# iden3/rapidsnark-old

Measured on AMD Instinct MI355X. Metric: Groth16 proofs/sec, higher is better.
Workload: dtype i64 (v_mad_i64_i32 column sums over 9x29-bit signed limbs, BN254 Fr/Fq)

## Files before the change

### include/zkhip.h

```cpp
#ifndef ZKHIP_H
#define ZKHIP_H

#include <stdint.h>
#include <stddef.h>

#ifdef __cplusplus
extern "C" {
#endif

typedef struct zk_prover zk_prover;

typedef struct zk_zkey_view {
    uint32_t nVars;
    uint32_t nPublic;
    uint32_t domainSize;
    uint64_t nCoefs;
    const void *vk_alpha1;
    const void *vk_beta1;
    const void *vk_beta2;
    const void *vk_delta1;
    const void *vk_delta2;
    const void *coefs;
    const void *pointsA;
    const void *pointsB1;
// ... 56 lines not shown
    uint32_t window_bits_w, windows_w;
    uint32_t precomputed_tables;
    uint32_t msm_a_b1_c_one_launch;
    uint32_t lanes;
    uint32_t follow_up_streams;
    uint32_t max_in_flight;
    uint32_t depth_host_witness;
    uint32_t depth_resident_witness;
    uint32_t batch;
    uint32_t shard_index, shard_count, chain_partitioned;
    uint64_t device_bytes_in_use;
    uint64_t device_bytes_total;
    uint64_t kernel_launches_last_proof;
    uint32_t table_rows_h, table_rows_w;
    uint32_t bucket_sets_h, bucket_sets_w;
} zk_prover_plan;
int zk_prover_info(zk_prover *p, zk_prover_plan *plan);
int zk_prove_msm_collect(zk_prover *p, zk_msm_sums *partial);
int zk_prove_batch_submit(zk_prover *p, const uint8_t *const *wtns, uint32_t count, const uint8_t *r32s, const uint8_t *s32s);
int zk_prove_batch_collect(zk_prover *p, zk_proof *out, uint32_t count);

int zk_prove_msm_dev(zk_prover *p, const void *d_wtns, zk_msm_sums *partial);
int zk_prove_msm(zk_prover *p, const uint8_t *wtns, zk_msm_sums *partial);
int zk_prove_finish(zk_prover *p, const zk_msm_sums *partials, uint32_t n_partials,
                    const uint8_t *r32, const uint8_t *s32, zk_proof *out);

typedef struct zk_multi_prover zk_multi_prover;
int zk_multi_prover_create(zk_multi_prover **out, const zk_zkey_view *zkey, const int32_t *devices, uint32_t n_devices,
                           const zk_opts *opts );
void zk_multi_prover_destroy(zk_multi_prover *mp);
// ... 103 lines not shown
```

### rapidsnark-old_amd/csrc/kernels.hpp

```cpp
#pragma once
#include <hip/hip_runtime.h>
#include <stdint.h>
#include "field.hpp"
#include "curve.hpp"

namespace zk {

void launch_fr_mul_vec(Fr *out, const Fr *a, const Fr *b, uint64_t n, hipStream_t s);
void launch_fq_mul_vec(Fq *out, const Fq *a, const Fq *b, uint64_t n, hipStream_t s);

struct CsrDev {
    const uint32_t *rowptr;
    const uint32_t *col;
    const Fr *val;
};
void launch_spmv_abc(Fr *a, Fr *b, Fr *c, CsrDev csr, const Fr *wtns, uint32_t n, hipStream_t s, uint32_t vectors = 1, uint64_t abc_stride = 0,
                     uint64_t wtns_stride = 0);
void launch_csr_build(uint32_t *rowptr, uint32_t *col, Fr *val, uint32_t *cursor, uint32_t *err, const uint8_t *records,
                      uint64_t nCoefs, uint32_t n, uint32_t nVars, uint32_t row_lo, uint32_t row_hi, hipStream_t s);
void launch_exclusive_scan_u32(uint32_t *out, const uint32_t *counts, uint32_t total, hipStream_t s);

struct TwEntry {
    uint32_t l[12];
};
// ... 2 lines not shown
    const TwEntry *fwd;
    const TwEntry *inv;
    const Fr *coset;
    const Fr *ninv;
};
struct NttPair {
    uint32_t L = 0, Lg = 0, m = 0;
    uint32_t ngroups = 0, g[2] = {0, 0};
    TwEntry *rfwd = nullptr, *rinv = nullptr;
    Fr *tinv = nullptr, *tfwd = nullptr, *dtab = nullptr, *t2inv = nullptr, *t2fwd = nullptr;
    NttPair() {}
    NttPair(const NttPair &) = delete;
    NttPair &operator=(const NttPair &) = delete;
    ~NttPair() { release(); }
    void build(uint32_t logn_global, uint32_t logn_local, uint32_t block_index, hipStream_t s, bool plain = false);
    void release();
};
bool ntt_pair_supported(uint32_t local_logn);
void launch_ntt_coset_pair(Fr *data, uint64_t stride_elems, uint32_t batch, const NttPair &t, hipStream_t s);
void launch_ntt_plain(Fr *out, Fr *data, uint64_t stride_elems, uint32_t batch, const NttPair &t, bool inverse, hipStream_t s);

void launch_ntt_build_tables(TwEntry *fwd, TwEntry *inv, Fr *coset, Fr *ninv, uint32_t logn, hipStream_t s);
#define NTT_FULL 0xffffffffu
void launch_ntt_dif_inverse(Fr *data, uint64_t stride_elems, uint32_t batch, const NttTables &t, hipStream_t s, uint32_t local_logn = NTT_FULL);
void launch_ntt_dit_forward(Fr *data, uint64_t stride_elems, uint32_t batch, const NttTables &t, hipStream_t s, const Fr *premul = nullptr,
                            uint32_t local_logn = NTT_FULL);
void launch_ntt_cross(bool inverse, const Fr *xb, uint64_t in_src_stride, uint64_t in_poly_stride, Fr *const out_base[8],
                      uint64_t out_poly_stride, uint64_t out_offset, uint32_t batch,
                      const NttTables &t, uint32_t log_shards, uint32_t rank, hipStream_t s);
void launch_chunk_scatter(Fr *const xb_of_gpu[8], const Fr *blockdata, uint32_t batch, uint32_t logn, uint32_t log_shards, uint32_t rank,
                          hipStream_t s);
void launch_chunk_pack(Fr *packed, const Fr *blockdata, uint32_t batch, uint32_t logn, uint32_t log_shards, hipStream_t s);
void launch_chunk_unpack(Fr *blockdata, const Fr *packed, uint32_t batch, uint32_t logn, uint32_t log_shards, hipStream_t s);
void launch_fr_to_internal(Fr *x, uint64_t n, int times, hipStream_t s);
// ... 81 lines not shown
```

### rapidsnark-old_amd/csrc/nttpair.hip

```cpp
#include <stdlib.h>
#include <string.h>
#include "kernels.hpp"
#include "hipcheck.hpp"
#include "common.hpp"
#include "field29.hpp"

namespace zk {

template <class F>
__device__ __forceinline__ F pload_el(const F *p) {
    const uint4 *q = reinterpret_cast<const uint4 *>(p);
    uint4 lo = q[0], hi = q[1];
    F r;
    r.v[0] = lo.x; r.v[1] = lo.y; r.v[2] = lo.z; r.v[3] = lo.w;
    r.v[4] = hi.x; r.v[5] = hi.y; r.v[6] = hi.z; r.v[7] = hi.w;
    return r;
}
template <class F>
__device__ __forceinline__ void pstore_el(F *p, const F &r) {
    uint4 *q = reinterpret_cast<uint4 *>(p);
    q[0] = make_uint4(r.v[0], r.v[1], r.v[2], r.v[3]);
    q[1] = make_uint4(r.v[4], r.v[5], r.v[6], r.v[7]);
}
__device__ __forceinline__ Fr29 pload_tw(const TwEntry *e) {
// ... 362 lines not shown
            const uint64_t i0 = i & (N1 - 1), k1 = pbrev((uint32_t)(i >> m), t);
            const uint64_t e = (i0 * k1) & (n - 1);
            pstore_el(tfwd + i, Fr29::store(Fr29::from_mont256(pfr_pow(s_wn, e))));
            pstore_el(tinv + i, Fr29::store(Fr29::from_mont256(Fr::mul(plain ? pfr_pow(s_wni, e) : Fr::mul(pfr_pow(s_wni, e), pfr_pow(s_w2n, k1)), s_kappa))));
        }
        if (t2fwd && i < (1ull << t)) {
            const uint32_t tb = t - ta;
            const uint64_t ja = i & ((1ull << ta) - 1), kb = pbrev((uint32_t)(i >> ta), tb);
            const uint64_t e = (ja * kb) & ((1ull << t) - 1);
            pstore_el(t2fwd + i, Fr29::store(Fr29::from_mont256(pfr_pow(s_wt, e))));
            pstore_el(t2inv + i, Fr29::store(Fr29::from_mont256(pfr_pow(s_wti, e))));
        }
    }
}

bool ntt_pair_supported(uint32_t local_logn) { return local_logn >= 3 && local_logn <= 27; }

void NttPair::build(uint32_t logn_global, uint32_t logn_local, uint32_t block_index, hipStream_t s, bool plain) {
    L = logn_local;
    Lg = logn_global;
    m = L < 11 ? L : 11;
    const uint32_t t = L - m;
    ngroups = t == 0 ? 0 : (t <= 11 ? 1 : 2);
    if (const char *e = probe_env("ZKHIP_NTT_SPLIT")) {
        if (atoi(e) == 2 && t >= 2) ngroups = 2;
    }
    g[0] = ngroups == 2 ? (t + 1) / 2 : t;
    g[1] = t - g[0];
    const uint64_t n = 1ull << L;
    auto dalloc = [&](void **p, size_t bytes) { ZK_HIP(hipMalloc(p, bytes ? bytes : 16)); };
// ... 5 lines not shown
        dalloc((void **)&tinv, n * sizeof(Fr));
        dalloc((void **)&tfwd, n * sizeof(Fr));
    }
    if (ngroups == 2) {
        dalloc((void **)&t2inv, ((size_t)1 << t) * sizeof(Fr));
        dalloc((void **)&t2fwd, ((size_t)1 << t) * sizeof(Fr));
    }
    const uint32_t lg = Lg - L;
    uint32_t rho = 0;
    for (uint32_t i = 0; i < lg; i++) rho |= ((block_index >> i) & 1u) << (lg - 1 - i);
    uint64_t grid = ((n > 2048 ? n : 2048) + 255) / 256;
    if (grid > 4096) grid = 4096;
    ZK_LAUNCH(k_pair_tables, dim3((uint32_t)grid), dim3(256), 0, s, rfwd, rinv, tinv, tfwd, dtab, t2inv, t2fwd, L, Lg, rho, m, g[0], plain ? 1u : 0u);
    ZK_LAUNCH_OK("ntt pair tables");
}
void NttPair::release() {
    for (void *p : {(void *)rfwd, (void *)rinv, (void *)tinv, (void *)tfwd, (void *)dtab, (void *)t2inv, (void *)t2fwd})
        if (p) (void)hipFree(p);
    rfwd = rinv = nullptr;
    tinv = tfwd = dtab = t2inv = t2fwd = nullptr;
}

static void lds_opt_in() {
    static PerDeviceOnce attr;
    if (!attr.need()) return;
    ZK_HIP(hipFuncSetAttribute((const void *)k_ntt_outer<true, 256>, hipFuncAttributeMaxDynamicSharedMemorySize, 160 * 1024));
    ZK_HIP(hipFuncSetAttribute((const void *)k_ntt_outer<false, 256>, hipFuncAttributeMaxDynamicSharedMemorySize, 160 * 1024));
    ZK_HIP(hipFuncSetAttribute((const void *)k_ntt_outer<true, 512>, hipFuncAttributeMaxDynamicSharedMemorySize, 160 * 1024));
    ZK_HIP(hipFuncSetAttribute((const void *)k_ntt_outer<false, 512>, hipFuncAttributeMaxDynamicSharedMemorySize, 160 * 1024));
    ZK_HIP(hipFuncSetAttribute((const void *)k_ntt_mid<0>, hipFuncAttributeMaxDynamicSharedMemorySize, 160 * 1024));
    ZK_HIP(hipFuncSetAttribute((const void *)k_ntt_mid<1>, hipFuncAttributeMaxDynamicSharedMemorySize, 160 * 1024));
// ... 57 lines not shown
            run_outer<true>(data, stride, batch, tb, tb.m + tb.g[0], tb.g[1], nullptr, 0, s);
            run_outer<true>(data, stride, batch, tb, tb.m, tb.g[0], tb.t2inv, t, s);
        } else if (tb.ngroups == 1) {
            run_outer<true>(data, stride, batch, tb, tb.m, t, nullptr, 0, s);
        }
    } else {
        if (tb.ngroups == 2) {
            run_outer<false>(data, stride, batch, tb, tb.m, tb.g[0], tb.t2fwd, t, s);
            run_outer<false>(data, stride, batch, tb, tb.m + tb.g[0], tb.g[1], nullptr, 0, s);
        } else if (tb.ngroups == 1) {
            run_outer<false>(data, stride, batch, tb, tb.m, t, nullptr, 0, s);
        }
    }
}

void launch_ntt_coset_pair(Fr *data, uint64_t stride, uint32_t batch, const NttPair &tb, hipStream_t s) {
    run_outer_passes<true>(data, stride, batch, tb, s);
    run_mid<0>(data, data, stride, batch, tb, s);
    run_outer_passes<false>(data, stride, batch, tb, s);
}

void launch_ntt_plain(Fr *out, Fr *data, uint64_t stride, uint32_t batch, const NttPair &tb, bool inverse, hipStream_t s) {
    if (inverse) {
        run_outer_passes<true>(data, stride, batch, tb, s);
        run_mid<1>(out, data, stride, batch, tb, s);
    } else {
        run_mid<2>(out, data, stride, batch, tb, s);
        run_outer_passes<false>(out, stride, batch, tb, s);
    }
}

}
```

### rapidsnark-old_amd/csrc/operators.hip

```cpp
#include "prover_internal.hpp"

static void need_device() { need_device_count(); }

template <class F>
static void mul_vec(uint8_t *out, const uint8_t *a, const uint8_t *b, uint64_t n, void (*launch)(F *, const F *, const F *, uint64_t, hipStream_t)) {
    need_device();
    if (!n) return;
    DevBuf<F> da, db;
    da.alloc(n);
    db.alloc(n);
    da.upload(a, n, 0);
    db.upload(b, n, 0);
    launch(da.p, da.p, db.p, n, 0);
    HIP_TRY(hipMemcpy(out, da.p, n * 32, hipMemcpyDeviceToHost));
}

struct Tables {
    DevBuf<TwEntry> fwd, inv;
    DevBuf<Fr> coset, ninv;
    NttTables t;
    void build(uint32_t logn) {
        uint64_t n = 1ull << logn;
        fwd.alloc(n > 1 ? n / 2 : 1);
        inv.alloc(n > 1 ? n / 2 : 1);
// ... 96 lines not shown
        need_device();
        uint32_t logn = ilog2_exact(n);
        if (logn > 27) throw std::invalid_argument("n exceeds 2^27");
        Tables tb;
        tb.build(logn);
        DevBuf<Fr> abc, hh;
        abc.alloc(3 * n);
        hh.alloc(n);
        HIP_TRY(hipMemcpy(abc.p, a, n * 32, hipMemcpyHostToDevice));
        HIP_TRY(hipMemcpy(abc.p + n, b, n * 32, hipMemcpyHostToDevice));
        launch_fr_mul_vec(abc.p + 2 * n, abc.p, abc.p + n, n, 0);
        launch_fr_to_internal(abc.p, 3 * n, 1, 0);
        if (ntt_pair_supported(logn) && !probe_env("ZKHIP_NTT_RADIX2")) {
            NttPair pr;
            pr.build(logn, logn, 0, 0);
            launch_ntt_coset_pair(abc.p, n, 3, pr, 0);
            HIP_TRY(hipStreamSynchronize(0));
        } else {
            launch_ntt_dif_inverse(abc.p, n, 3, tb.t, 0);
            launch_ntt_dit_forward(abc.p, n, 3, tb.t, 0, tb.coset.p);
        }
        launch_abc_to_h(hh.p, abc.p, abc.p + n, abc.p + 2 * n, n, 0);
        HIP_TRY(hipMemcpy(h, hh.p, n * 32, hipMemcpyDeviceToHost));
    });
}

}

template <class AffT, class XT, class AccT>
static void msm_generic(uint8_t *out, const uint8_t *bases, const uint8_t *scalars, uint64_t n, bool g2) {
    need_device();
// ... 103 lines not shown
```

### rapidsnark-old_amd/csrc/prover_create.hip

```cpp
#include "prover_internal.hpp"

__attribute__((constructor)) static void zk_default_hw_queues() { setenv("GPU_MAX_HW_QUEUES", "16", 0); }

namespace zkp {

void alloc_slot(zk_prover *p, int i) {
    zk_prover::ProofSlot &q = p->slot[i];
    if (q.allocated) return;
    const uint64_t nv = p->sv.size();
    q.sort_w.alloc(nv, p->wbits, p->table_mode, p->batch);
    const MsmPlan pw = q.sort_w.plan, ph = p->sort_h.plan;
    const uint64_t tbw = q.sort_w.total_buckets(), tbh = p->sort_h.total_buckets();
    q.buckets_g1.alloc(3 * tbw + tbh);
    q.buckets_g2.alloc(tbw);
    q.scratch_g1.alloc(msm_reduce_scratch_points(3, pw) + msm_reduce_scratch_points(1, ph));
    const uint64_t ew = (uint64_t)pw.sets * msm_wsum_rc(pw), eh = (uint64_t)ph.sets * msm_wsum_rc(ph);
    q.wsum_g1.alloc(3 * ew + eh);
    q.scratch_g2.alloc(msm_reduce_scratch_points(1, pw));
    q.wsum_g2.alloc(ew);
    const uint64_t slots = msm_accum_workspace_slots(q.sort_w.max_entries()), slots_h = msm_accum_workspace_slots(p->sort_h.max_entries());
    q.acc_stride = slots;
    q.acc_ws_g1_all.alloc(3 * slots + slots_h);
    q.acc_ws_g2.alloc(slots);
    q.acc_key_all.alloc(4 * slots + slots_h);
    q.acc_flag_all.alloc(4 * slots + slots_h);
    for (int m = 0; m < 5; m++) {
        const uint64_t at = m < 3 ? m * slots : (m == 3 ? 3 * slots : 3 * slots + slots_h);
        if (m < 4) q.acc_ws_g1[m] = q.acc_ws_g1_all.p + at;
        q.acc_key[m] = q.acc_key_all.p + at;
        q.acc_flag[m] = q.acc_flag_all.p + at;
    }
    q.w1_bytes = (size_t)(3 * ew + eh) * sizeof(G1XYZZ);
    q.w2_bytes = (size_t)ew * sizeof(G2XYZZ);
    if (!q.w1) HIP_TRY(hipHostMalloc((void **)&q.w1, q.w1_bytes, hipHostMallocDefault));
    if (!q.w2) HIP_TRY(hipHostMalloc((void **)&q.w2, q.w2_bytes, hipHostMallocDefault));
    for (auto &e : q.ev_l1)
        if (!e) HIP_TRY(hipEventCreateWithFlags(&e, hipEventDisableTiming));
    for (hipEvent_t *e : {&q.ev_fork, &q.ev_join, &q.ev_sortw, &q.ev_main, &q.ev_done, &q.ev_chain})
        if (!*e) HIP_TRY(hipEventCreateWithFlags(e, hipEventDisableTiming));
    for (auto &e : q.ev_tail)
        if (!e) HIP_TRY(hipEventCreateWithFlags(&e, hipEventDisableTiming));
    for (auto &e : q.ev)
        if (!e) HIP_TRY(hipEventCreate(&e));
    q.have_events = true;
    q.allocated = true;
}

void ensure_witness_buffer(zk_prover *p, zk_prover::ProofSlot &q) {
    if (!q.wtns_dev.p) q.wtns_dev.alloc((uint64_t)p->nVars * p->batch);
    if (!q.ev_h2d) HIP_TRY(hipEventCreateWithFlags(&q.ev_h2d, hipEventDisableTiming));
    if (!q.ev_h2d_start) HIP_TRY(hipEventCreate(&q.ev_h2d_start));
}

// ... 83 lines not shown
            {
                const char *e = getenv("ZKHIP_TAIL");
                int ntail = e ? atoi(e) : (p->shard_count > 1 ? 2 : 0);
                if (getenv("ZKHIP_SERIAL")) ntail = 0;
                if (ntail != 0 && ntail != 5) ntail = 2;
                p->tail_streams = ntail;
                if (ntail) {
                    int lo_pr = 0, hi_pr = 0;
                    HIP_TRY(hipDeviceGetStreamPriorityRange(&lo_pr, &hi_pr));
                    for (int i = 0; i < ntail; i++) HIP_TRY(hipStreamCreateWithPriority(&p->tail_pool[i], hipStreamNonBlocking, hi_pr));
                    for (int m = 0; m < 5; m++) p->tail[m] = ntail == 5 ? p->tail_pool[m] : p->tail_pool[(m == 2 || m == 3) ? 1 : 0];
                }
            }
            HIP_TRY(hipStreamCreateWithFlags(&p->stream_fin, hipStreamNonBlocking));
            HIP_TRY(hipStreamCreateWithFlags(&p->stream_h2d, hipStreamNonBlocking));
        } catch (...) {
            side.err = std::current_exception();
        }
    });
    p->wbits = (wbits == 0 && (p->flags & ZK_FLAG_SPARSE_WITNESS) && (p->flags & ZK_FLAG_PRECOMP) && p->logn > 18) ? 16u : wbits;
    hipStream_t s = p->stream;
    clk.lap("device + first stream", s);
    StreamUploader up(s);

    p->sv = shard_slice(nV, p->shard_index, p->shard_count);
    p->sh = shard_slice(n, p->shard_index, p->shard_count);
    p->part = (p->flags & ZK_FLAG_PARTITIONED_CHAIN) != 0 && p->shard_count > 1;
    if (p->part) {
        uint32_t lg = 0;
        while ((1u << lg) < p->shard_count) lg++;
// ... 25 lines not shown
        clk.lap("coefficient records upload", s);
        launch_csr_build(p->csr_rowptr.p, p->csr_col.p, p->csr_val.p, cursor.p, err.p, raw.p, nnz, z->domainSize, z->nVars,
                         p->part ? (uint32_t)p->sh.lo : 0u, p->part ? (uint32_t)p->sh.hi : z->domainSize, s);
        launch_fr_to_internal(p->csr_val.p, nnz, 2, s);
        uint32_t bad = 0;
        HIP_TRY(hipMemcpyAsync(&bad, err.p, 4, hipMemcpyDeviceToHost, s));
        HIP_TRY(hipStreamSynchronize(s));
        if (bad) throw std::invalid_argument("zkey coefficient record out of range");
        clk.lap("CSR build (device)", s);
    }

    {
        const uint32_t local_logn = p->logn - p->log_shards_chain();
        const bool pair = ntt_pair_supported(local_logn) && !probe_env("ZKHIP_NTT_RADIX2");
        if (pair) p->pair.build(p->logn, local_logn, p->part ? p->shard_index : 0u, s);
        if (!pair || p->part) {
            p->tw_fwd.alloc(n > 1 ? n / 2 : 1);
            p->tw_inv.alloc(n > 1 ? n / 2 : 1);
            if (!pair) p->tw_coset.alloc(n);
            p->tw_ninv.alloc(1);
            launch_ntt_build_tables(p->tw_fwd.p, p->tw_inv.p, p->tw_coset.p, p->tw_ninv.p, p->logn, s);
        }
    }
    clk.lap("twiddle tables", s);

    const uint64_t nv = p->sv.size(), nh = p->sh.size();
    p->precomp = (p->flags & ZK_FLAG_PRECOMP) != 0;
    p->table_mode = (p->flags & ZK_FLAG_PRECOMP_HALF) ? 2u : p->precomp ? 1u : 0u;
    p->sort_h.alloc(nh, wbits, p->table_mode, p->batch);
    alloc_slot(p.get(), 0);
// ... 179 lines not shown
        o.lanes = (uint32_t)p->lanes;
        o.follow_up_streams = (uint32_t)p->tail_streams;
        o.max_in_flight = ZK_MAX_IN_FLIGHT;
        const bool small = p->logn < 19, mid = p->logn <= 22 && p->shard_count == 1;
        o.depth_host_witness = small ? ZK_MAX_IN_FLIGHT : mid ? 6u : 3u;
        o.depth_resident_witness = small ? ZK_MAX_IN_FLIGHT : mid ? 6u : 2u;
        o.batch = p->batch;
        o.shard_index = p->shard_index; o.shard_count = p->shard_count; o.chain_partitioned = p->part ? 1u : 0u;
        {
            DeviceGuard g(p->device);
            size_t fr = 0, tot = 0;
            HIP_TRY(hipMemGetInfo(&fr, &tot));
            o.device_bytes_in_use = tot - fr; o.device_bytes_total = tot;
        }
        o.kernel_launches_last_proof = p->launches_last_proof;
        const uint32_t nb = plan->size < sizeof o ? plan->size : (uint32_t)sizeof o;
        o.size = nb;
        memcpy(plan, &o, nb);
    });
}

}
```

### rapidsnark-old_amd/csrc/prover_internal.hpp

```cpp
#pragma once
#include <hip/hip_runtime.h>
#include <string.h>
#include <stdio.h>
#include <stdlib.h>
#include <chrono>
#include <sys/random.h>
#include <string>
#include <vector>
#include <atomic>
#include <condition_variable>
#include <deque>
#include <map>
#include <mutex>
#include <thread>
#include <memory>
#include <stdexcept>
#include <exception>
#include <functional>

#include "../../include/zkhip.h"
#include "common.hpp"
#include "hipcheck.hpp"
#include "kernels.hpp"
#include "tail_pool.hpp"
// ... 144 lines not shown
struct zk_prover {
    int device = 0;
    uint32_t flags = 0;
    uint32_t nVars = 0, nPublic = 0, domainSize = 0, logn = 0;
    uint64_t nCoefs = 0;
    uint32_t shard_index = 0, shard_count = 1;
    uint8_t vk_alpha1[64], vk_beta1[64], vk_beta2[128], vk_delta1[64], vk_delta2[128];
    hipStream_t stream = nullptr, stream2 = nullptr;
    std::mutex mtx, cmtx, sync_mtx;

    DevBuf<uint32_t> csr_rowptr, csr_col;
    DevBuf<Fr> csr_val;
    DevBuf<TwEntry> tw_fwd, tw_inv;
    DevBuf<Fr> tw_coset, tw_ninv;
    NttPair pair;
    Slice sv, sh;
    uint32_t c_idx_min = 0;
    bool precomp = false;
    uint32_t table_mode = 0;
    DevBuf<G1Affine> ptsA, ptsB1, ptsC, ptsH;
    DevBuf<G2Affine> ptsB2;

    DevBuf<Fr> abc, h;
    SortBufs sort_h;
    struct ProofSlot {
        bool allocated = false, busy = false;
        bool use_tails = true;
        uint32_t l1_chunk_min = 0, l1_chunk_max = 0;
        SortBufs sort_w;
        DevBuf<G1Acc> buckets_g1;
        DevBuf<G2Acc> buckets_g2;
        DevBuf<G1Acc> scratch_g1, acc_ws_g1_all;
        G1Acc *acc_ws_g1[4] = {nullptr, nullptr, nullptr, nullptr};
        DevBuf<uint32_t> acc_key_all, acc_flag_all;
        uint32_t *acc_key[5] = {nullptr}, *acc_flag[5] = {nullptr};
        uint64_t acc_stride = 0;
        DevBuf<G2Acc> scratch_g2, acc_ws_g2;
        DevBuf<G1XYZZ> wsum_g1;
        DevBuf<G2XYZZ> wsum_g2;
        hipEvent_t ev_l1[5] = {nullptr, nullptr, nullptr, nullptr, nullptr};
        hipEvent_t ev_fork = nullptr, ev_join = nullptr, ev_sortw = nullptr, ev_main = nullptr, ev_done = nullptr, ev_chain = nullptr;
        bool zeroed = false;
        bool defer_w = false;
        hipEvent_t ev_tail[5] = {nullptr, nullptr, nullptr, nullptr, nullptr};
        hipEvent_t ev[20] = {};
        bool have_events = false;
        uint8_t *w1 = nullptr, *w2 = nullptr;
        size_t w1_bytes = 0, w2_bytes = 0;
        DevBuf<Fr> wtns_dev;
        uint8_t *wtns_pin = nullptr;
        uint8_t *pin_ring = nullptr;
        StageJob stage[ZK_MAX_BATCH];
        StageJob stage_chunk[16];
        hipEvent_t ev_h2d_b = nullptr;
        hipEvent_t ev_h2d = nullptr, ev_h2d_start = nullptr;
        uint8_t r32[ZK_MAX_BATCH][32], s32[ZK_MAX_BATCH][32];
        bool have_r = false, have_s = false;
// ... 15 lines not shown
            acc_key_all.release(); acc_flag_all.release(); scratch_g2.release(); acc_ws_g2.release();
            wsum_g1.release(); wsum_g2.release(); wtns_dev.release();
            if (w1) { (void)hipHostFree(w1); w1 = nullptr; }
            if (w2) { (void)hipHostFree(w2); w2 = nullptr; }
            if (wtns_pin) { (void)hipHostFree(wtns_pin); wtns_pin = nullptr; }
            if (pin_ring) { (void)hipHostFree(pin_ring); pin_ring = nullptr; }
            if (gexec) { (void)hipGraphExecDestroy(gexec); gexec = nullptr; }
            if (graph) { (void)hipGraphDestroy(graph); graph = nullptr; }
            graph_wtns = nullptr;
        }
        ~ProofSlot() {
            if (gexec) (void)hipGraphExecDestroy(gexec);
            if (graph) (void)hipGraphDestroy(graph);
            if (ev_gdone) (void)hipEventDestroy(ev_gdone);
            for (auto &e : ev_l1) if (e) (void)hipEventDestroy(e);
            for (hipEvent_t e : {ev_fork, ev_join, ev_sortw, ev_main, ev_done, ev_chain}) if (e) (void)hipEventDestroy(e);
            for (auto &e : ev_tail) if (e) (void)hipEventDestroy(e);
            for (auto &e : ev) if (e) (void)hipEventDestroy(e);
            if (w1) (void)hipHostFree(w1);
            if (w2) (void)hipHostFree(w2);
            if (wtns_pin) (void)hipHostFree(wtns_pin);
            if (pin_ring) (void)hipHostFree(pin_ring);
            if (ev_h2d) (void)hipEventDestroy(ev_h2d);
            if (ev_h2d_b) (void)hipEventDestroy(ev_h2d_b);
            if (ev_h2d_start) (void)hipEventDestroy(ev_h2d_start);
        }
    };
    ProofSlot slot[ZK_MAX_IN_FLIGHT];
    uint32_t next_submit = 0, next_collect = 0, in_flight = 0;
    uint32_t ring = ZK_MAX_IN_FLIGHT;
    uint32_t batch = 1;
// ... 38 lines not shown
    Fr *abc_use = nullptr, *xb_use = nullptr;
    Fr *pk_use = nullptr;
    Fr *peer_abc[8] = {nullptr}, *peer_xb[8] = {nullptr};
    bool have_peers = false;
    int phase_open = -1, phase_next = 0;
    hipEvent_t ev_ext_in = nullptr, ev_ext_out = nullptr;
    uint32_t log_shards_chain() const { return part ? log_shards : 0; }
    hipStream_t tail_pool[5] = {nullptr, nullptr, nullptr, nullptr, nullptr};
    hipStream_t tail[5] = {nullptr, nullptr, nullptr, nullptr, nullptr};
    int tail_streams = 0;
    bool use_graph = false;
    bool capturing = false;
    bool batch_abc = false;
    hipStream_t stream_fin = nullptr;
    hipStream_t stream_h2d = nullptr;

    double timings[ZK_T_COUNT] = {0};
    uint32_t accum_launches = 0;
    uint64_t launches_at_front = 0, launches_last_proof = 0;

    ~zk_prover() {
        for (auto &x : extra)
            if (x && x->stream) { (void)hipStreamSynchronize(x->stream); (void)hipStreamSynchronize(x->stream2); }
        for (hipStream_t st : {stream_h2d, stream, stream2, tail_pool[0], tail_pool[1], tail_pool[2], tail_pool[3], tail_pool[4], stream_fin})
            if (st) (void)hipStreamSynchronize(st);
        if (ev_ext_in) (void)hipEventDestroy(ev_ext_in);
        if (ev_ext_out) (void)hipEventDestroy(ev_ext_out);
        if (stream_h2d) (void)hipStreamDestroy(stream_h2d);
        if (stream_fin) (void)hipStreamDestroy(stream_fin);
        for (hipStream_t st : tail_pool)
            if (st) (void)hipStreamDestroy(st);
        if (stream2 && stream2 != stream) (void)hipStreamDestroy(stream2);
        if (stream) (void)hipStreamDestroy(stream);
    }
};

namespace zkp {

inline void need_device_count() {
    int ndev = 0;
    HIP_TRY(hipGetDeviceCount(&ndev));
    if (ndev <= 0) throw std::runtime_error("no HIP device available (libzkhip has no CPU fallback)");
}

// ... 77 lines not shown
```

### rapidsnark-old_amd/csrc/prover_pipeline.hip

```cpp
#include "prover_internal.hpp"

namespace {
struct StagePool {
    struct Seg { uint8_t *dst; const uint8_t *src; size_t len; std::atomic<int> *left; };
    std::mutex m;
    std::condition_variable cv, done;
    std::deque<Seg> q;
    std::vector<std::thread> th;
    bool stop = false;
    StagePool() {
        for (int i = 0; i < 4; i++) th.emplace_back([this] { run(); });
    }
    ~StagePool() {
        {
            std::lock_guard<std::mutex> lk(m);
            stop = true;
        }
        cv.notify_all();
        for (auto &t : th) t.join();
    }
    void run() {
        for (;;) {
            Seg s;
            {
// ... 97 lines not shown
    if (count < p->batch) HIP_TRY(hipMemsetAsync((uint8_t *)q.wtns_dev.p + (size_t)count * bytes, 0, (size_t)(p->batch - count) * bytes, sh));
    HIP_TRY(hipEventRecord(q.ev_h2d, sh));
    if (tm) HIP_TRY(hipEventRecord(q.ev[12], sh));
    return q.wtns_dev.p;
}
static const Fr *upload_witness(zk_prover *p, zk_prover::ProofSlot &q, const uint8_t *h_wtns, hipEvent_t src_ready = nullptr) {
    return upload_witnesses(p, q, &h_wtns, 1, src_ready);
}

namespace {

struct PhaseCtx {
    zk_prover *p;
    zk_prover::ProofSlot &q;
    hipStream_t s, s2, sf;
    hipStream_t tail[5] = {nullptr, nullptr, nullptr, nullptr, nullptr};
    int ntails = 0;
    Fr *abc, *h;
    SortBufs *sort_h;
    bool tm;
    uint32_t tbw, tbh, Ww;
    uint64_t ew, eh;
    MsmPlan pw;
    G1Acc *bA, *bB1, *bC, *bH;
    PhaseCtx(zk_prover *p_, int si) : p(p_), q(p_->slot[si]) {
        const int lane = si % p->lanes;
        if (lane == 0) {
            s = p->stream; s2 = p->stream2; sf = p->stream_fin;
            if (q.use_tails) {
                for (int m = 0; m < 5; m++) tail[m] = p->tail[m];
                ntails = p->tail_streams;
            }
            abc = p->abc_use; h = p->h.p; sort_h = &p->sort_h;
        } else {
            zk_prover::LaneExtra &x = *p->extra[lane - 1];
            x.ensure();
            s = x.stream; s2 = x.stream2; sf = x.stream;
            abc = x.abc.p; h = x.h.p; sort_h = &x.sort_h;
        }
        tm = (p->flags & ZK_FLAG_TIMINGS) != 0;
        tbw = q.sort_w.total_buckets(); tbh = p->sort_h.total_buckets();
        ew = q.sort_w.max_entries(); eh = p->sort_h.max_entries();
        pw = q.sort_w.plan; Ww = pw.sets * msm_wsum_rc(pw);
        bA = q.buckets_g1.p; bB1 = bA + tbw; bC = bB1 + tbw; bH = bC + tbw;
    }
    void mark(int i) const { if (tm) HIP_TRY(hipEventRecord(q.ev[i], s)); }
    AccumTail tail_of(int m) const { AccumTail t; t.stream = tail[m]; t.l1_done = q.ev_l1[m]; t.buckets_zeroed = q.zeroed; t.chunk_min = q.l1_chunk_min; t.chunk_max = q.l1_chunk_max; return t; }
    hipStream_t after(int m, hipStream_t own) const { return tail[m] ? tail[m] : own; }
    NttTables tables() const { return NttTables{p->logn, p->tw_fwd.p, p->tw_inv.p, p->tw_coset.p, p->tw_ninv.p}; }
};


static bool lone_order(const zk_prover *p) {
    static const int forced = [] { const char *e = probe_env("ZKHIP_LONE_ORDER"); return e ? atoi(e) : -1; }();
    return forced > 0 && p->shard_count == 1 && !p->part;
}

static void enqueue_witness_msms(zk_prover *p, PhaseCtx &c) {
    zk_prover::ProofSlot &q = c.q;
    hipStream_t s2 = c.s2;
    const bool tails = c.ntails != 0;
    const bool tm = c.tm;
    const uint32_t tbw = c.tbw, Ww = c.Ww;
    const uint64_t ew = c.ew;
    const MsmPlan pw = c.pw;
    static const uint32_t g2_aside_maxlog = [] { const char *e = probe_env("ZKHIP_G2_ASIDE_MAXLOG"); return e ? (uint32_t)atoi(e) : 21u; }();
    const bool g2_aside = !tails && c.sf != s2 && c.sf != c.s && p->in_flight == 0 && !p->capturing && !p->use_graph &&
                          p->sv.size() <= ((uint64_t)1 << g2_aside_maxlog);
    AccumTail t4 = c.tail_of(4);
    if (g2_aside) t4.stream = c.sf;
    launch_msm_accum_g2(q.buckets_g2.p, q.sort_w.offsets.p, q.sort_w.entries.p, p->ptsB2.p, 0, 0, tbw, ew, q.acc_ws_g2.p, q.acc_key[4], q.acc_flag[4], s2, tm ? &q.ev[10] : nullptr, t4);
    if (tails) launch_msm_reduce_g2(q.wsum_g2.p, q.scratch_g2.p, q.buckets_g2.p, 1, pw, c.tail[4]);
    else if (g2_aside) launch_msm_reduce_g2(q.wsum_g2.p, q.scratch_g2.p, q.buckets_g2.p, 1, pw, c.sf);
    if (p->batch_abc) {
        AccumBatch b;
        memset(&b, 0, sizeof b);
        b.n = 3;
        b.points[0] = p->ptsA.p; b.points[1] = p->ptsB1.p; b.points[2] = p->ptsC.p;
        static const bool one_table = probe_env("ZKHIP_PROBE_ONE_TABLE") != nullptr;
        if (one_table) b.points[1] = b.points[2] = p->ptsA.p;
        b.idx_min[2] = b.idx_sub[2] = p->c_idx_min;
        b.bucket_stride = tbw;
        b.ws_stride = q.acc_stride;
// ... 28 lines not shown
    if (p->in_flight == 0 && !p->capturing) p->next_submit = p->next_collect = 0;
    const int si = (int)(p->next_submit % p->ring);
    alloc_slot(p, si);
    if (!p->capturing) p->slot[si].use_tails = p->in_flight > 0 || p->use_graph;
    if (!p->capturing) {
        static const uint32_t thr_min = [] { const char *e = probe_env("ZKHIP_L1_CHUNK_MIN_BUSY"); return e ? (uint32_t)atoi(e) : 128u; }();
        static const uint32_t thr_log = [] { const char *e = probe_env("ZKHIP_L1_CHUNK_MIN_BUSY_LOG"); return e ? (uint32_t)atoi(e) : 17u; }();
        static const uint32_t thr_max = [] { const char *e = probe_env("ZKHIP_L1_CHUNK_MAX_BUSY"); return e ? (uint32_t)atoi(e) : 1280u; }();
        static const bool shards_too = [] { const char *e = probe_env("ZKHIP_L1_BUSY_SHARDS"); return e ? atoi(e) != 0 : true; }();
        uint32_t lg_sh = 0;
        while ((1u << (lg_sh + 1)) <= p->shard_count) lg_sh++;
        const bool busy = p->in_flight > 0 && !p->use_graph && ((p->shard_count == 1 && !p->part) || shards_too) && p->batch == 1 && p->logn >= thr_log + lg_sh;
        p->slot[si].l1_chunk_min = busy ? thr_min : 0u;
        p->slot[si].l1_chunk_max = busy ? thr_max : 0u;
    }
    PhaseCtx c(p, si);
    zk_prover::ProofSlot &q = c.q;
    if (!p->capturing) p->launches_at_front = g_kernel_launches.load(std::memory_order_relaxed);
    bool staged = h_wtns != nullptr;
    q.count = 1;
    if (bi) {
        if (bi->count < 1 || bi->count > p->batch) throw std::invalid_argument("batch submission: between 1 and opts.batch witnesses");
        d_wtns = upload_witnesses(p, q, bi->wtns, bi->count, src_ready);
        staged = true;
        q.count = bi->count;
        r32 = bi->r32s;
        s32 = bi->s32s;
    } else if (staged) {
        d_wtns = upload_witness(p, q, h_wtns, src_ready);
    } else if (p->batch > 1) {
        d_wtns = upload_witnesses(p, q, nullptr, 1, src_ready, d_wtns);
        staged = true;
// ... 59 lines not shown
    if (done) HIP_TRY(hipEventRecord(done, c.s));
    p->phase_next = inverse ? 2 : 4;
}

void phase_local(zk_prover *p) {
    if (p->phase_open < 0 || p->phase_next != 2) throw std::invalid_argument("chain phases out of order");
    DeviceGuard g(p->device);
    PhaseCtx c(p, p->phase_open);
    const uint32_t local_logn = p->logn - p->log_shards_chain();
    const uint64_t nl = p->nloc;
    NttTables tb = c.tables();
    const bool a2a = p->part && !p->have_peers;
    if (a2a) launch_chunk_unpack(c.abc, p->pk_use, 3, p->logn, p->log_shards, c.s);
    if (p->pair.L) {
        static const bool skip_ntt = probe_env("ZKHIP_PROBE_SKIP_NTT") != nullptr;
        launch_ntt_coset_pair(c.abc, nl, (skip_ntt ? 1 : 3) * c.q.count, p->pair, c.s);
    } else {
        launch_ntt_dif_inverse(c.abc, nl, 3 * c.q.count, tb, c.s, local_logn);
        launch_ntt_dit_forward(c.abc, nl, 3 * c.q.count, tb, c.s, p->tw_coset.p + (p->part ? p->sh.lo : 0), local_logn);
    }
    if (a2a) launch_chunk_pack(p->pk_use, c.abc, 3, p->logn, p->log_shards, c.s);
    if (c.q.defer_w) {
        HIP_TRY(hipEventRecord(c.q.ev_chain, c.s));
        HIP_TRY(hipStreamWaitEvent(c.s2, c.q.ev_chain, 0));
        enqueue_witness_msms(p, c);
        c.q.defer_w = false;
    }
    p->phase_next = p->part ? 3 : 4;
}

void phase_back(zk_prover *p) {
    if (p->phase_open < 0 || p->phase_next != 4) throw std::invalid_argument("chain phases out of order");
    DeviceGuard g(p->device);
    PhaseCtx c(p, p->phase_open);
    zk_prover::ProofSlot &q = c.q;
    hipStream_t s = c.s;
    const uint64_t nl = p->nloc;
    Fr *abc = c.abc;
    if (p->part && !p->have_peers) launch_chunk_unpack(abc, p->pk_use, 3, p->logn, p->log_shards, s);
    launch_abc_to_h(c.h, abc, abc + nl, abc + 2 * nl, nl, s, q.count, 3 * nl);
    if (q.count < p->batch) HIP_TRY(hipMemsetAsync(c.h + nl * q.count, 0, (size_t)(p->batch - q.count) * nl * sizeof(Fr), s));
    c.mark(2);
    c.sort_h->run(c.h + (p->part ? 0 : p->sh.lo), s);
    c.mark(3);
    launch_msm_accum_g1(c.bH, c.sort_h->offsets.p, c.sort_h->entries.p, p->ptsH.p, 0, 0, c.tbh, c.eh, q.acc_ws_g1[3], q.acc_key[3], q.acc_flag[3], s, c.tm ? &q.ev[17] : nullptr, c.tail_of(3));
    c.mark(4);
    launch_msm_reduce_g1(q.wsum_g1.p + 3 * c.Ww, q.scratch_g1.p + msm_reduce_scratch_points(3, c.pw), c.bH, 1, p->sort_h.plan, c.after(3, s));
    if (!p->batch_abc) {
    HIP_TRY(hipStreamWaitEvent(s, q.ev_sortw, 0));
    launch_msm_accum_g1(c.bC, q.sort_w.offsets.p, q.sort_w.entries.p, p->ptsC.p, p->c_idx_min, p->c_idx_min, c.tbw, c.ew, q.acc_ws_g1[2], q.acc_key[2], q.acc_flag[2], s, c.tm ? &q.ev[15] : nullptr, c.tail_of(2));
    launch_msm_reduce_g1(q.wsum_g1.p + 2 * c.Ww, q.scratch_g1.p + msm_reduce_scratch_points(2, c.pw), c.bC, 1, c.pw, c.after(2, s));
    }
    c.mark(5);
    HIP_TRY(hipEventRecord(q.ev_main, s));

    hipStream_t sf = c.sf;
    HIP_TRY(hipStreamWaitEvent(sf, q.ev_main, 0));
    HIP_TRY(hipStreamWaitEvent(sf, q.ev_join, 0));
    for (int i = 0; i < c.ntails; i++) {
// ... 335 lines not shown
```

### rapidsnark-old_amd/lib.py

```python
import ctypes as C
import os

import numpy as np

_HERE = os.path.dirname(os.path.abspath(__file__))
_LIB = None


class ZkHipError(RuntimeError):
    pass


def library_path():
    return os.environ.get("ZKHIP_LIB") or os.path.join(_HERE, "libzkhip.so")


class zk_zkey_view(C.Structure):
    _fields_ = [("nVars", C.c_uint32), ("nPublic", C.c_uint32), ("domainSize", C.c_uint32), ("nCoefs", C.c_uint64),
                ("vk_alpha1", C.c_void_p), ("vk_beta1", C.c_void_p), ("vk_beta2", C.c_void_p),
                ("vk_delta1", C.c_void_p), ("vk_delta2", C.c_void_p), ("coefs", C.c_void_p),
                ("pointsA", C.c_void_p), ("pointsB1", C.c_void_p), ("pointsB2", C.c_void_p),
                ("pointsC", C.c_void_p), ("pointsH", C.c_void_p),
                ("coefs_bytes", C.c_uint64), ("pointsA_bytes", C.c_uint64), ("pointsB1_bytes", C.c_uint64),
                ("pointsB2_bytes", C.c_uint64), ("pointsC_bytes", C.c_uint64), ("pointsH_bytes", C.c_uint64)]
# ... 8 lines not shown
    _fields_ = [("A", C.c_uint8 * 64), ("B", C.c_uint8 * 128), ("C", C.c_uint8 * 64)]


class zk_msm_sums(C.Structure):
    _fields_ = [("pih", C.c_uint8 * 64), ("pi_a", C.c_uint8 * 64), ("pib1", C.c_uint8 * 64),
                ("pi_b", C.c_uint8 * 128), ("pi_c", C.c_uint8 * 64)]


class zk_prover_plan(C.Structure):
    _fields_ = [("size", C.c_uint32), ("window_bits_h", C.c_uint32), ("windows_h", C.c_uint32), ("window_bits_w", C.c_uint32),
                ("windows_w", C.c_uint32), ("precomputed_tables", C.c_uint32), ("msm_a_b1_c_one_launch", C.c_uint32), ("lanes", C.c_uint32),
                ("follow_up_streams", C.c_uint32), ("max_in_flight", C.c_uint32), ("depth_host_witness", C.c_uint32),
                ("depth_resident_witness", C.c_uint32), ("batch", C.c_uint32), ("shard_index", C.c_uint32), ("shard_count", C.c_uint32),
                ("chain_partitioned", C.c_uint32), ("device_bytes_in_use", C.c_uint64), ("device_bytes_total", C.c_uint64),
                ("kernel_launches_last_proof", C.c_uint64), ("table_rows_h", C.c_uint32), ("table_rows_w", C.c_uint32),
                ("bucket_sets_h", C.c_uint32), ("bucket_sets_w", C.c_uint32)]


class zk_r1cs_view(C.Structure):
    _fields_ = [("nWires", C.c_uint32), ("nPubOut", C.c_uint32), ("nPubIn", C.c_uint32), ("nPrvIn", C.c_uint32),
                ("nConstraints", C.c_uint32), ("constraints", C.c_void_p), ("constraints_bytes", C.c_uint64)]


class zk_r1cs_report(C.Structure):
    _fields_ = [("size", C.c_uint32), ("failed", C.c_uint64), ("first_failed", C.c_uint32), ("a", C.c_uint8 * 32),
                ("b", C.c_uint8 * 32), ("c", C.c_uint8 * 32), ("one_ok", C.c_uint32), ("first_unreduced", C.c_uint32)]


class zk_ptau_view(C.Structure):
    _fields_ = [("power", C.c_uint32), ("alpha1", C.c_void_p), ("beta1", C.c_void_p), ("beta2", C.c_void_p),
                ("lagrange_g1", C.c_void_p), ("lagrange_g2", C.c_void_p), ("lagrange_alpha_g1", C.c_void_p), ("lagrange_beta_g1", C.c_void_p),
# ... 341 lines not shown
```

Measured before the change: 30.49.

## Add high-priority lone stream for forward NTT and H chain, regroup NTT passes

For single-proof, unsharded, non-graph runs, the forward half of the coset NTT, the abc-to-h step and the H digit sort move onto a new high-priority stream, linked to the main stream by events. The G2 MSM may also be placed on the side stream in this mode. A regrouped NTT plan splits a single-group pass into two groups with its own twiddle table, built when the group size is 11 or the env mode asks for it. The goal is to get the latency-critical H chain scheduled ahead of the concurrent witness MSMs and to use smaller NTT passes, at the cost of extra events, stream contention and extra table memory.

Measured after the change: 30.27. No clear change (-0.7%).

```diff
diff --git a/include/zkhip.h b/include/zkhip.h
--- a/include/zkhip.h
+++ b/include/zkhip.h
@@ -94,6 +94,12 @@
     uint64_t kernel_launches_last_proof;
     uint32_t table_rows_h, table_rows_w;
     uint32_t bucket_sets_h, bucket_sets_w;
+    uint32_t lone_plan;
+    uint32_t lone_plan_min_log2n;
+    uint32_t last_proof_lone;
+    uint32_t last_proof_ntt_groups;
+    uint32_t last_proof_ntt_pass_threads;
+    uint32_t reserved0;
 } zk_prover_plan;
 int zk_prover_info(zk_prover *p, zk_prover_plan *plan);
 int zk_prove_msm_collect(zk_prover *p, zk_msm_sums *partial);
diff --git a/rapidsnark-old_amd/csrc/kernels.hpp b/rapidsnark-old_amd/csrc/kernels.hpp
--- a/rapidsnark-old_amd/csrc/kernels.hpp
+++ b/rapidsnark-old_amd/csrc/kernels.hpp
@@ -40,10 +40,13 @@
     NttPair &operator=(const NttPair &) = delete;
     ~NttPair() { release(); }
     void build(uint32_t logn_global, uint32_t logn_local, uint32_t block_index, hipStream_t s, bool plain = false);
+    bool build_regrouped(const NttPair &base, hipStream_t s);
+    bool borrowed = false;
     void release();
 };
 bool ntt_pair_supported(uint32_t local_logn);
-void launch_ntt_coset_pair(Fr *data, uint64_t stride_elems, uint32_t batch, const NttPair &t, hipStream_t s);
+void launch_ntt_coset_pair(Fr *data, uint64_t stride_elems, uint32_t batch, const NttPair &t, hipStream_t s, hipStream_t s_fwd = nullptr,
+                           hipEvent_t hop = nullptr);
 void launch_ntt_plain(Fr *out, Fr *data, uint64_t stride_elems, uint32_t batch, const NttPair &t, bool inverse, hipStream_t s);
 
 void launch_ntt_build_tables(TwEntry *fwd, TwEntry *inv, Fr *coset, Fr *ninv, uint32_t logn, hipStream_t s);
diff --git a/rapidsnark-old_amd/csrc/nttpair.hip b/rapidsnark-old_amd/csrc/nttpair.hip
--- a/rapidsnark-old_amd/csrc/nttpair.hip
+++ b/rapidsnark-old_amd/csrc/nttpair.hip
@@ -400,6 +400,23 @@
     }
 }
 
+__global__ __launch_bounds__(256) void k_pair_tables_t2(Fr *t2inv, Fr *t2fwd, uint32_t t, uint32_t ta) {
+    __shared__ Fr s_wt, s_wti;
+    if (threadIdx.x == 0) {
+        s_wt = pfr_root(t);
+        s_wti = Fr::inv(s_wt);
+    }
+    __syncthreads();
+    const uint64_t st = (uint64_t)gridDim.x * blockDim.x;
+    for (uint64_t i = (uint64_t)blockIdx.x * blockDim.x + threadIdx.x; i < (1ull << t); i += st) {
+        const uint32_t tb = t - ta;
+        const uint64_t ja = i & ((1ull << ta) - 1), kb = pbrev((uint32_t)(i >> ta), tb);
+        const uint64_t e = (ja * kb) & ((1ull << t) - 1);
+        pstore_el(t2fwd + i, Fr29::store(Fr29::from_mont256(pfr_pow(s_wt, e))));
+        pstore_el(t2inv + i, Fr29::store(Fr29::from_mont256(pfr_pow(s_wti, e))));
+    }
+}
+
 bool ntt_pair_supported(uint32_t local_logn) { return local_logn >= 3 && local_logn <= 27; }
 
 void NttPair::build(uint32_t logn_global, uint32_t logn_local, uint32_t block_index, hipStream_t s, bool plain) {
@@ -435,7 +452,26 @@
     ZK_LAUNCH(k_pair_tables, dim3((uint32_t)grid), dim3(256), 0, s, rfwd, rinv, tinv, tfwd, dtab, t2inv, t2fwd, L, Lg, rho, m, g[0], plain ? 1u : 0u);
     ZK_LAUNCH_OK("ntt pair tables");
 }
+bool NttPair::build_regrouped(const NttPair &base, hipStream_t s) {
+    release();
+    const uint32_t t = base.L - base.m;
+    if (!base.L || t < 2) return false;
+    L = base.L; Lg = base.Lg; m = base.m;
+    ngroups = 2;
+    g[0] = (t + 1) / 2;
+    g[1] = t - g[0];
+    borrowed = true;
+    rfwd = base.rfwd; rinv = base.rinv; tinv = base.tinv; tfwd = base.tfwd; dtab = base.dtab;
+    ZK_HIP(hipMalloc((void **)&t2inv, ((size_t)1 << t) * sizeof(Fr)));
+    ZK_HIP(hipMalloc((void **)&t2fwd, ((size_t)1 << t) * sizeof(Fr)));
+    const uint64_t grid = (((uint64_t)1 << t) + 255) / 256;
+    ZK_LAUNCH(k_pair_tables_t2, dim3((uint32_t)(grid > 4096 ? 4096 : grid)), dim3(256), 0, s, t2inv, t2fwd, t, g[0]);
+    ZK_LAUNCH_OK("ntt pair tables (regrouped)");
+    return true;
+}
 void NttPair::release() {
+    if (borrowed) rfwd = rinv = nullptr, tinv = tfwd = dtab = nullptr;
+    borrowed = false;
     for (void *p : {(void *)rfwd, (void *)rinv, (void *)tinv, (void *)tfwd, (void *)dtab, (void *)t2inv, (void *)t2fwd})
         if (p) (void)hipFree(p);
     rfwd = rinv = nullptr;
@@ -523,9 +559,14 @@
     }
 }
 
-void launch_ntt_coset_pair(Fr *data, uint64_t stride, uint32_t batch, const NttPair &tb, hipStream_t s) {
+void launch_ntt_coset_pair(Fr *data, uint64_t stride, uint32_t batch, const NttPair &tb, hipStream_t s, hipStream_t s_fwd, hipEvent_t hop) {
     run_outer_passes<true>(data, stride, batch, tb, s);
     run_mid<0>(data, data, stride, batch, tb, s);
+    if (s_fwd && s_fwd != s) {
+        ZK_HIP(hipEventRecord(hop, s));
+        ZK_HIP(hipStreamWaitEvent(s_fwd, hop, 0));
+        s = s_fwd;
+    }
     run_outer_passes<false>(data, stride, batch, tb, s);
 }
 
diff --git a/rapidsnark-old_amd/csrc/operators.hip b/rapidsnark-old_amd/csrc/operators.hip
--- a/rapidsnark-old_amd/csrc/operators.hip
+++ b/rapidsnark-old_amd/csrc/operators.hip
@@ -134,7 +134,10 @@
         if (ntt_pair_supported(logn) && !probe_env("ZKHIP_NTT_RADIX2")) {
             NttPair pr;
             pr.build(logn, logn, 0, 0);
-            launch_ntt_coset_pair(abc.p, n, 3, pr, 0);
+            NttPair two;
+            const char *lp = getenv("ZKHIP_LONE_PLAN");
+            const bool regroup = lp && atoi(lp) > 1 && pr.ngroups == 1 && two.build_regrouped(pr, 0);
+            launch_ntt_coset_pair(abc.p, n, 3, regroup ? two : pr, 0);
             HIP_TRY(hipStreamSynchronize(0));
         } else {
             launch_ntt_dif_inverse(abc.p, n, 3, tb.t, 0);
diff --git a/rapidsnark-old_amd/csrc/prover_create.hip b/rapidsnark-old_amd/csrc/prover_create.hip
--- a/rapidsnark-old_amd/csrc/prover_create.hip
+++ b/rapidsnark-old_amd/csrc/prover_create.hip
@@ -36,7 +36,7 @@
     if (!q.w2) HIP_TRY(hipHostMalloc((void **)&q.w2, q.w2_bytes, hipHostMallocDefault));
     for (auto &e : q.ev_l1)
         if (!e) HIP_TRY(hipEventCreateWithFlags(&e, hipEventDisableTiming));
-    for (hipEvent_t *e : {&q.ev_fork, &q.ev_join, &q.ev_sortw, &q.ev_main, &q.ev_done, &q.ev_chain})
+    for (hipEvent_t *e : {&q.ev_fork, &q.ev_join, &q.ev_sortw, &q.ev_main, &q.ev_done, &q.ev_chain, &q.ev_lone})
         if (!*e) HIP_TRY(hipEventCreateWithFlags(e, hipEventDisableTiming));
     for (auto &e : q.ev_tail)
         if (!e) HIP_TRY(hipEventCreateWithFlags(&e, hipEventDisableTiming));
@@ -150,6 +150,17 @@
             }
             HIP_TRY(hipStreamCreateWithFlags(&p->stream_fin, hipStreamNonBlocking));
             HIP_TRY(hipStreamCreateWithFlags(&p->stream_h2d, hipStreamNonBlocking));
+            {
+                const char *e = getenv("ZKHIP_LONE_PLAN");
+                const int mode = e ? atoi(e) : 1;
+                if (mode > 0 && p->shard_count == 1 && p->batch == 1 && !getenv("ZKHIP_SERIAL")) {
+                    int lo_pr = 0, hi_pr = 0;
+                    HIP_TRY(hipDeviceGetStreamPriorityRange(&lo_pr, &hi_pr));
+                    const char *pe = probe_env("ZKHIP_LONE_PRIO");
+                    HIP_TRY(hipStreamCreateWithPriority(&p->stream_lone, hipStreamNonBlocking, pe && atoi(pe) == 0 ? lo_pr : hi_pr));
+                    p->lone_mode = mode > 1 ? 2u : 1u;
+                }
+            }
         } catch (...) {
             side.err = std::current_exception();
         }
@@ -205,6 +216,14 @@
         const uint32_t local_logn = p->logn - p->log_shards_chain();
         const bool pair = ntt_pair_supported(local_logn) && !probe_env("ZKHIP_NTT_RADIX2");
         if (pair) p->pair.build(p->logn, local_logn, p->part ? p->shard_index : 0u, s);
+        {
+            const char *e = getenv("ZKHIP_LONE_PLAN");
+            const int mode = e ? atoi(e) : 1;
+            const bool unsharded = p->shard_count == 1 && p->batch == 1 && !getenv("ZKHIP_SERIAL");
+            const char *ge = probe_env("ZKHIP_LONE_GROUPS");
+            const bool regroup = !(ge && atoi(ge) == 1);
+            if (pair && unsharded && regroup && p->pair.ngroups == 1 && (mode > 1 || (mode == 1 && p->pair.g[0] == 11))) p->pair_lone.build_regrouped(p->pair, s);
+        }
         if (!pair || p->part) {
             p->tw_fwd.alloc(n > 1 ? n / 2 : 1);
             p->tw_inv.alloc(n > 1 ? n / 2 : 1);
@@ -414,6 +433,8 @@
             o.device_bytes_in_use = tot - fr; o.device_bytes_total = tot;
         }
         o.kernel_launches_last_proof = p->launches_last_proof;
+        o.lone_plan = p->lone_mode; o.lone_plan_min_log2n = p->lone_min_logn;
+        o.last_proof_lone = p->last_lone; o.last_proof_ntt_groups = p->last_ntt_groups; o.last_proof_ntt_pass_threads = p->last_ntt_threads;
         const uint32_t nb = plan->size < sizeof o ? plan->size : (uint32_t)sizeof o;
         o.size = nb;
         memcpy(plan, &o, nb);
diff --git a/rapidsnark-old_amd/csrc/prover_internal.hpp b/rapidsnark-old_amd/csrc/prover_internal.hpp
--- a/rapidsnark-old_amd/csrc/prover_internal.hpp
+++ b/rapidsnark-old_amd/csrc/prover_internal.hpp
@@ -182,6 +182,7 @@
     DevBuf<TwEntry> tw_fwd, tw_inv;
     DevBuf<Fr> tw_coset, tw_ninv;
     NttPair pair;
+    NttPair pair_lone;
     Slice sv, sh;
     uint32_t c_idx_min = 0;
     bool precomp = false;
@@ -207,8 +208,9 @@
         DevBuf<G1XYZZ> wsum_g1;
         DevBuf<G2XYZZ> wsum_g2;
         hipEvent_t ev_l1[5] = {nullptr, nullptr, nullptr, nullptr, nullptr};
-        hipEvent_t ev_fork = nullptr, ev_join = nullptr, ev_sortw = nullptr, ev_main = nullptr, ev_done = nullptr, ev_chain = nullptr;
+        hipEvent_t ev_fork = nullptr, ev_join = nullptr, ev_sortw = nullptr, ev_main = nullptr, ev_done = nullptr, ev_chain = nullptr, ev_lone = nullptr;
         bool zeroed = false;
+        bool lone = false;
         bool defer_w = false;
         hipEvent_t ev_tail[5] = {nullptr, nullptr, nullptr, nullptr, nullptr};
         hipEvent_t ev[20] = {};
@@ -254,7 +256,7 @@
             if (graph) (void)hipGraphDestroy(graph);
             if (ev_gdone) (void)hipEventDestroy(ev_gdone);
             for (auto &e : ev_l1) if (e) (void)hipEventDestroy(e);
-            for (hipEvent_t e : {ev_fork, ev_join, ev_sortw, ev_main, ev_done, ev_chain}) if (e) (void)hipEventDestroy(e);
+            for (hipEvent_t e : {ev_fork, ev_join, ev_sortw, ev_main, ev_done, ev_chain, ev_lone}) if (e) (void)hipEventDestroy(e);
             for (auto &e : ev_tail) if (e) (void)hipEventDestroy(e);
             for (auto &e : ev) if (e) (void)hipEventDestroy(e);
             if (w1) (void)hipHostFree(w1);
@@ -323,6 +325,9 @@
     bool batch_abc = false;
     hipStream_t stream_fin = nullptr;
     hipStream_t stream_h2d = nullptr;
+    hipStream_t stream_lone = nullptr;
+    uint32_t lone_mode = 0, lone_min_logn = 20;
+    uint32_t last_lone = 0, last_ntt_groups = 0, last_ntt_threads = 0;
 
     double timings[ZK_T_COUNT] = {0};
     uint32_t accum_launches = 0;
@@ -331,12 +336,13 @@
     ~zk_prover() {
         for (auto &x : extra)
             if (x && x->stream) { (void)hipStreamSynchronize(x->stream); (void)hipStreamSynchronize(x->stream2); }
-        for (hipStream_t st : {stream_h2d, stream, stream2, tail_pool[0], tail_pool[1], tail_pool[2], tail_pool[3], tail_pool[4], stream_fin})
+        for (hipStream_t st : {stream_h2d, stream_lone, stream, stream2, tail_pool[0], tail_pool[1], tail_pool[2], tail_pool[3], tail_pool[4], stream_fin})
             if (st) (void)hipStreamSynchronize(st);
         if (ev_ext_in) (void)hipEventDestroy(ev_ext_in);
         if (ev_ext_out) (void)hipEventDestroy(ev_ext_out);
         if (stream_h2d) (void)hipStreamDestroy(stream_h2d);
         if (stream_fin) (void)hipStreamDestroy(stream_fin);
+        if (stream_lone) (void)hipStreamDestroy(stream_lone);
         for (hipStream_t st : tail_pool)
             if (st) (void)hipStreamDestroy(st);
         if (stream2 && stream2 != stream) (void)hipStreamDestroy(stream2);
diff --git a/rapidsnark-old_amd/csrc/prover_pipeline.hip b/rapidsnark-old_amd/csrc/prover_pipeline.hip
--- a/rapidsnark-old_amd/csrc/prover_pipeline.hip
+++ b/rapidsnark-old_amd/csrc/prover_pipeline.hip
@@ -135,6 +135,7 @@
     zk_prover *p;
     zk_prover::ProofSlot &q;
     hipStream_t s, s2, sf;
+    hipStream_t sc;
     hipStream_t tail[5] = {nullptr, nullptr, nullptr, nullptr, nullptr};
     int ntails = 0;
     Fr *abc, *h;
@@ -159,13 +160,15 @@
             s = x.stream; s2 = x.stream2; sf = x.stream;
             abc = x.abc.p; h = x.h.p; sort_h = &x.sort_h;
         }
+        sc = q.lone ? p->stream_lone : s;
         tm = (p->flags & ZK_FLAG_TIMINGS) != 0;
         tbw = q.sort_w.total_buckets(); tbh = p->sort_h.total_buckets();
         ew = q.sort_w.max_entries(); eh = p->sort_h.max_entries();
         pw = q.sort_w.plan; Ww = pw.sets * msm_wsum_rc(pw);
         bA = q.buckets_g1.p; bB1 = bA + tbw; bC = bB1 + tbw; bH = bC + tbw;
     }
-    void mark(int i) const { if (tm) HIP_TRY(hipEventRecord(q.ev[i], s)); }
+    void mark(int i, hipStream_t on = nullptr) const { if (tm) HIP_TRY(hipEventRecord(q.ev[i], on ? on : s)); }
+    const NttPair &pair() const { return q.lone && p->pair_lone.L ? p->pair_lone : p->pair; }
     AccumTail tail_of(int m) const { AccumTail t; t.stream = tail[m]; t.l1_done = q.ev_l1[m]; t.buckets_zeroed = q.zeroed; t.chunk_min = q.l1_chunk_min; t.chunk_max = q.l1_chunk_max; return t; }
     hipStream_t after(int m, hipStream_t own) const { return tail[m] ? tail[m] : own; }
     NttTables tables() const { return NttTables{p->logn, p->tw_fwd.p, p->tw_inv.p, p->tw_coset.p, p->tw_ninv.p}; }
@@ -186,8 +189,9 @@
     const uint64_t ew = c.ew;
     const MsmPlan pw = c.pw;
     static const uint32_t g2_aside_maxlog = [] { const char *e = probe_env("ZKHIP_G2_ASIDE_MAXLOG"); return e ? (uint32_t)atoi(e) : 21u; }();
+    static const bool lone_aside = [] { const char *e = probe_env("ZKHIP_LONE_G2_ASIDE"); return e ? atoi(e) != 0 : true; }();
     const bool g2_aside = !tails && c.sf != s2 && c.sf != c.s && p->in_flight == 0 && !p->capturing && !p->use_graph &&
-                          p->sv.size() <= ((uint64_t)1 << g2_aside_maxlog);
+                          (p->sv.size() <= ((uint64_t)1 << g2_aside_maxlog) || (q.lone && lone_aside));
     AccumTail t4 = c.tail_of(4);
     if (g2_aside) t4.stream = c.sf;
     launch_msm_accum_g2(q.buckets_g2.p, q.sort_w.offsets.p, q.sort_w.entries.p, p->ptsB2.p, 0, 0, tbw, ew, q.acc_ws_g2.p, q.acc_key[4], q.acc_flag[4], s2, tm ? &q.ev[10] : nullptr, t4);
@@ -246,8 +250,18 @@
         p->slot[si].l1_chunk_min = busy ? thr_min : 0u;
         p->slot[si].l1_chunk_max = busy ? thr_max : 0u;
     }
+    if (!p->capturing) {
+        p->slot[si].lone = p->lone_mode && p->stream_lone && p->in_flight == 0 && !p->use_graph && p->shard_count == 1 && !p->part &&
+                           p->batch == 1 && si % p->lanes == 0 && (p->lone_mode > 1 || p->logn >= p->lone_min_logn);
+    }
     PhaseCtx c(p, si);
     zk_prover::ProofSlot &q = c.q;
+    if (!p->capturing) {
+        const NttPair &np = c.pair();
+        p->last_lone = q.lone ? 1u : 0u;
+        p->last_ntt_groups = np.L ? np.ngroups : 0u;
+        p->last_ntt_threads = np.L && np.ngroups ? (np.g[0] == 11 || np.g[1] == 11 ? 512u : 256u) : 0u;
+    }
     if (!p->capturing) p->launches_at_front = g_kernel_launches.load(std::memory_order_relaxed);
     bool staged = h_wtns != nullptr;
     q.count = 1;
@@ -337,14 +351,18 @@
     if (a2a) launch_chunk_unpack(c.abc, p->pk_use, 3, p->logn, p->log_shards, c.s);
     if (p->pair.L) {
         static const bool skip_ntt = probe_env("ZKHIP_PROBE_SKIP_NTT") != nullptr;
-        launch_ntt_coset_pair(c.abc, nl, (skip_ntt ? 1 : 3) * c.q.count, p->pair, c.s);
+        launch_ntt_coset_pair(c.abc, nl, (skip_ntt ? 1 : 3) * c.q.count, c.pair(), c.s, c.sc, c.q.ev_lone);
     } else {
         launch_ntt_dif_inverse(c.abc, nl, 3 * c.q.count, tb, c.s, local_logn);
-        launch_ntt_dit_forward(c.abc, nl, 3 * c.q.count, tb, c.s, p->tw_coset.p + (p->part ? p->sh.lo : 0), local_logn);
+        if (c.sc != c.s) {
+            HIP_TRY(hipEventRecord(c.q.ev_lone, c.s));
+            HIP_TRY(hipStreamWaitEvent(c.sc, c.q.ev_lone, 0));
+        }
+        launch_ntt_dit_forward(c.abc, nl, 3 * c.q.count, tb, c.sc, p->tw_coset.p + (p->part ? p->sh.lo : 0), local_logn);
     }
     if (a2a) launch_chunk_pack(p->pk_use, c.abc, 3, p->logn, p->log_shards, c.s);
     if (c.q.defer_w) {
-        HIP_TRY(hipEventRecord(c.q.ev_chain, c.s));
+        HIP_TRY(hipEventRecord(c.q.ev_chain, c.sc));
         HIP_TRY(hipStreamWaitEvent(c.s2, c.q.ev_chain, 0));
         enqueue_witness_msms(p, c);
         c.q.defer_w = false;
@@ -361,11 +379,15 @@
     const uint64_t nl = p->nloc;
     Fr *abc = c.abc;
     if (p->part && !p->have_peers) launch_chunk_unpack(abc, p->pk_use, 3, p->logn, p->log_shards, s);
-    launch_abc_to_h(c.h, abc, abc + nl, abc + 2 * nl, nl, s, q.count, 3 * nl);
-    if (q.count < p->batch) HIP_TRY(hipMemsetAsync(c.h + nl * q.count, 0, (size_t)(p->batch - q.count) * nl * sizeof(Fr), s));
-    c.mark(2);
-    c.sort_h->run(c.h + (p->part ? 0 : p->sh.lo), s);
-    c.mark(3);
+    launch_abc_to_h(c.h, abc, abc + nl, abc + 2 * nl, nl, c.sc, q.count, 3 * nl);
+    if (q.count < p->batch) HIP_TRY(hipMemsetAsync(c.h + nl * q.count, 0, (size_t)(p->batch - q.count) * nl * sizeof(Fr), c.sc));
+    c.mark(2, c.sc);
+    c.sort_h->run(c.h + (p->part ? 0 : p->sh.lo), c.sc);
+    c.mark(3, c.sc);
+    if (c.sc != s) {
+        HIP_TRY(hipEventRecord(q.ev_chain, c.sc));
+        HIP_TRY(hipStreamWaitEvent(s, q.ev_chain, 0));
+    }
     launch_msm_accum_g1(c.bH, c.sort_h->offsets.p, c.sort_h->entries.p, p->ptsH.p, 0, 0, c.tbh, c.eh, q.acc_ws_g1[3], q.acc_key[3], q.acc_flag[3], s, c.tm ? &q.ev[17] : nullptr, c.tail_of(3));
     c.mark(4);
     launch_msm_reduce_g1(q.wsum_g1.p + 3 * c.Ww, q.scratch_g1.p + msm_reduce_scratch_points(3, c.pw), c.bH, 1, p->sort_h.plan, c.after(3, s));
diff --git a/rapidsnark-old_amd/lib.py b/rapidsnark-old_amd/lib.py
--- a/rapidsnark-old_amd/lib.py
+++ b/rapidsnark-old_amd/lib.py
@@ -46,7 +46,9 @@
                 ("depth_resident_witness", C.c_uint32), ("batch", C.c_uint32), ("shard_index", C.c_uint32), ("shard_count", C.c_uint32),
                 ("chain_partitioned", C.c_uint32), ("device_bytes_in_use", C.c_uint64), ("device_bytes_total", C.c_uint64),
                 ("kernel_launches_last_proof", C.c_uint64), ("table_rows_h", C.c_uint32), ("table_rows_w", C.c_uint32),
-                ("bucket_sets_h", C.c_uint32), ("bucket_sets_w", C.c_uint32)]
+                ("bucket_sets_h", C.c_uint32), ("bucket_sets_w", C.c_uint32), ("lone_plan", C.c_uint32), ("lone_plan_min_log2n", C.c_uint32),
+                ("last_proof_lone", C.c_uint32), ("last_proof_ntt_groups", C.c_uint32), ("last_proof_ntt_pass_threads", C.c_uint32),
+                ("reserved0", C.c_uint32)]
 
 
 class zk_r1cs_view(C.Structure):
```
